# ghy1228/LDPC_Error_Floor

Measured on AMD Instinct MI355X. Metric: decoded codewords/sec, wman N576 R3/4, 20 NMS iters, higher is better.
Workload: dtype i32

## Files before the change

include/ldpc_nms.h:

```cpp
#ifndef LDPC_NMS_H
#define LDPC_NMS_H

#include <stdint.h>

#ifdef __cplusplus
extern "C" {
#endif

#define LDPC_NMS_ABI_VERSION 3

typedef struct ldpc_graph ldpc_graph;
typedef struct ldpc_ctx ldpc_ctx;

enum ldpc_status {
    LDPC_OK = 0,
    LDPC_ERR_ARG = -1,
    LDPC_ERR_HIP = -2,
    LDPC_ERR_OOM = -3,
    LDPC_ERR_STATE = -4,
    LDPC_ERR_UNSUPPORTED = -5
};

enum ldpc_decoding_type {
    LDPC_DEC_SP = 0,
// ... 31 lines not shown
int ldpc_abi_version(void);
const char* ldpc_status_string(int status);

int ldpc_graph_create(const int32_t* proto, int32_t M, int32_t N, int32_t z, int32_t device,
                      ldpc_graph** out);
int ldpc_graph_destroy(ldpc_graph* g);
int ldpc_graph_query(const ldpc_graph* g, int32_t* dims);

int ldpc_weights_set(ldpc_graph* g, int32_t T, const float* alpha, const float* alpha_ucn,
                     const float* beta);

int ldpc_ctx_create(ldpc_graph* g, int64_t B_max, int32_t T_max, ldpc_ctx** out);
int ldpc_ctx_destroy(ldpc_ctx* c);

int ldpc_decode(ldpc_ctx* c, const float* llr_dev, int64_t B, const ldpc_decode_params* p,
                const ldpc_decode_outputs* o, void* stream);

int ldpc_kernel_info(const ldpc_ctx* c, const ldpc_decode_params* p, int64_t* bytes_per_cw,
                     char* name, int32_t name_len);

int ldpc_ctx_last_kernel(const ldpc_ctx* c, char* name, int32_t name_len);

int ldpc_ctx_last_frozen(const ldpc_ctx* c);

int ldpc_channel_awgn(float* llr_dev, int64_t B, int32_t n_vars, double sigma, uint64_t seed,
                      int64_t offset, int32_t decoding_type, int32_t q_bit, int32_t punct_start,
                      int32_t punct_end, int32_t short_start, int32_t short_end, float clip_llr,
                      void* stream);

typedef struct ldpc_channel_params {
    double sigma;
    uint64_t seed;
    int64_t offset;
    int32_t punct_start, punct_end, short_start, short_end;
    int32_t reserved[4];
} ldpc_channel_params;

int ldpc_decode_awgn(ldpc_ctx* ctx, int64_t B, const ldpc_decode_params* params,
                     const ldpc_channel_params* channel, const ldpc_decode_outputs* outputs,
                     void* stream);

int ldpc_awgn_in_kernel(const ldpc_ctx* ctx, const ldpc_decode_params* params, int32_t has_short,
                        int32_t app);

typedef struct ldpc_es_outputs {
    int32_t size;
// ... 101 lines not shown
```

include/ldpc_nms_debug.h:

```cpp
#ifndef LDPC_NMS_DEBUG_H
#define LDPC_NMS_DEBUG_H

#include <stdint.h>

#include "ldpc_nms.h"

#ifdef __cplusplus
extern "C" {
#endif

int ldpc_debug_bs_bounds(const int32_t* proto, int32_t M, int32_t N, int32_t z, int32_t T,
                         int32_t mode, int32_t alpha_uniform, int32_t beta_uniform, float clip,
                         int32_t flags, int32_t* violations, char* msg, int32_t msg_len);

int ldpc_debug_bs_frozen(const int32_t* proto, int32_t M, int32_t N, int32_t z, int32_t T, int32_t mode,
                         int32_t alpha_uniform, int32_t beta_uniform, int32_t ucn, int32_t kind,
                         float clip, int32_t* plan, int32_t* frozen, int32_t n, char* names,
                         int32_t names_len);

int ldpc_debug_events_out(ldpc_ctx* ctx, const uint32_t* planes_dev, const uint32_t* bad_dev, int64_t B,
                          int32_t target_bits, const uint8_t* n_iter_dev, int32_t T,
                          const ldpc_event_outputs* outputs, void* stream);

#ifdef __cplusplus
}
#endif

#endif
```

ldpc_error_floor_amd/csrc/ldpc_bs.hip:

```cpp
#include <algorithm>
#include <array>
#include <cmath>
#include <cstdio>
#include <cstdlib>
#include <cstring>
#include <functional>
#include <string>
#include <utility>
#include <vector>

#include "ldpc_bs_host.h"

namespace ldpc {
namespace bs {

__global__ void k_bs_tables(const float* __restrict__ alpha, const float* __restrict__ alpha_ucn,
                            const float* __restrict__ beta, const int32_t* __restrict__ row_ptr,
                            int T, int E, int N, int arows, int ar, int bcols, float step, float inv,
                            int qmax, float cu, uint32_t* alut, uint32_t* blut) {
    const int f = blockIdx.x * blockDim.x + threadIdx.x;
    const int na = T * ar, nbt = T * bcols;
    if (f >= na + nbt) return;
    int g[16];
    uint32_t* out;
// ... 700 lines not shown
    a.cn_lanes = p.cn_lanes;
    a.cn_dmin = p.cn_dmin;
    a.fold_wave = p.cn_lanes < 64 * p.nw ? (uint32_t)(p.nw - 1) : (p.nw > 1 ? 1u : 0u);
    a.inv = 1.0f / step;
    a.cu = p.cu > 0.f ? p.cu : -1.f;
    a.qmax = bs_qmax(r.mode);
    a.ucn = p.ucn ? 1 : 0;
    a.ucn_iter = g.w_ucn_iter;
    a.beta_id = g.w_beta_id_mask;
    a.row_ptr = g.row_ptr;
    a.z = g.z;
    a.vn_tab = gt;
    const size_t nvt = (size_t)k.VPL * 64 * p.nw * VNW;
    a.vn_wdeg = reinterpret_cast<const int32_t*>(gt + nvt);
    a.row_lay = a.vn_wdeg + 3 * (size_t)k.VPL * p.nw;
    a.cn_chunk = a.row_lay + 2 * (size_t)g.M;
    a.cn_hd = reinterpret_cast<const uint32_t*>(a.cn_chunk + (size_t)p.nw * k.CPL);
    a.alut = alut;
    a.blut = blut;
    a.arows = p.arows;
    a.bcols = p.bcols;
    a.btid = (bs_qmax(r.mode) == QMAX && !getenv("LDPC_BS_NOBFIX")) ? g.beta_tid : nullptr;
    a.btid_n = g.N;
    a.counters = o.counters;
    a.flags = o.flags;
    a.bad = o.bad;
    a.iter_wrong = r.es ? nullptr : b.iter_wrong;
    a.hdx = o.hdx;
    bs_stagger(k.VPL > 1 || k.CPL > 1, &a.stagger, &a.stagger_n);
    a.off_slots = p.off_slots;
    a.off_pad = p.off_pad;
    a.off_zero = p.off_zero;
    a.off_red = p.off_red;
    a.off_alut = p.off_alut;
    a.off_blut = p.off_blut;
    a.off_hdz = p.off_hdz;
    a.off_hdl = p.off_hdl;
    a.off_ch = p.off_ch;
    if (const char* e = getenv("LDPC_DIAG_ABLATE")) a.ablate = atoi(e);
    const int npacks = (int)((b.B + PACK - 1) / PACK);
    int grid = -1;
    if (const char* e = getenv("LDPC_BS_GRID")) grid = std::max(atoi(e), 0);
    a.ticket = nullptr;
    if (bs_loops(k)) {
        const char* e = getenv("LDPC_BS_TICKETS");
        if (e ? atoi(e) != 0 : true) {
// ... 50 lines not shown
            fprintf(f, "bs_wg_launch inst %d T %d B %lld packs %d q8 %d frozen %d tickets %d\n"
                    "# bs_wg wg packs rt_entry rt_exit clk_entry clk_exit hw_id xcc_id   (rt: 100 MHz ticks, clk: shader clocks)\n",
                    p.inst, b.T, (long long)b.B, npacks, b.q8 != nullptr, (int)frozen, tickets);
            for (int w = 0; w < npacks; ++w) {
                const unsigned long long* r = rec.data() + (size_t)BS_WG_REC * w;
                if (!r[0]) continue;
                fprintf(f, "bs_wg %d %llu %llu %llu %llu %llu %08llx %llu\n", w, r[0], r[1], r[2], r[3], r[4],
                        r[5] & 0xFFFFFFFFull, r[5] >> 32);
            }
            fclose(f);
        }
    }
    return st;
#else
    return kLaunch[p.inst](a, npacks, p.nw, lds, s, src, grid, ws.bs_resident);
#endif
}

int bs_decode(const DevGraph& g, const Bufs& b, FusedWorkspace& ws, const float* llr, const BsReq& r,
              const BsOut& o, hipStream_t s) {
    bool to_bsc;
    BsPlan p = bs_route(g, r, &to_bsc);
    ws.bs_frozen = false;
    if (!p.ok) return to_bsc ? bsc_decode(g, b, ws, llr, r, o, s) : LDPC_ERR_UNSUPPORTED;
    const bool frozen = bs_frozen_fit(g, p, r, o.hdx != nullptr || o.hdw != nullptr);
    return bs_run(g, b, ws, p, llr, r, o, frozen, s);
}

}

namespace ldpc {
namespace bs {
struct BoundsReport {
    int violations = 0;
    std::string first;
    void fail(const char* what, long long idx, long long lim) {
        if (violations++ == 0) {
            char buf[160];
            snprintf(buf, sizeof(buf), "%s: index %lld outside [0, %lld)", what, idx, lim);
            first = buf;
        }
    }
    void in(const char* what, long long idx, long long lim) {
        if (idx < 0 || idx >= lim) fail(what, idx, lim);
    }
    void lds(const char* what, long long a, long long n, long long lo, long long hi) {
// ... 238 lines not shown
```

ldpc_error_floor_amd/csrc/ldpc_bs_kernel.h:

```cpp
#pragma once
#include <type_traits>
#include <cstdint>

#include "ldpc_beta_tabs.h"
#include "ldpc_fused.h"
#include "ldpc_fused5_kernel.h"
#include "ldpc_bitplane.h"
#include "ldpc_bs_frozen.h"

namespace ldpc {
namespace bs {

constexpr int PACK = 32;
constexpr int SLOT_W = 5;
constexpr int SLOT_B = SLOT_W * 4;
constexpr int LUT_W = 64;
constexpr int BLUT_W = LUT_W + 4;
constexpr int QMAX = 15;
constexpr size_t BS_LDS_MAX = 160 * 1024;

struct BsInst { int D, DV, LPC, VPL, CPL; bool UCN, BIG, PK; int WPE; bool ES = false; };
constexpr BsInst kBsInst[] = {
    {15, 6, 4, 1, 1, false, false, true, 8},
    {16, 8, 4, 1, 1, false, false, true, 8},
// ... 403 lines not shown
        int la[4];
        awgn_levels4b(g, bucket, thi, tlo, (uint32_t)v, gq, la);
        uint32_t w = word(la);
        if (sh) {
            int lb[4];
            awgn_levels4b(g, bucket, thi, tlo, (uint32_t)v, gq + 1, lb);
            w = __builtin_amdgcn_alignbyte(word(lb), w, (uint32_t)sh);
        }
        D[i] = w;
    }
}
__device__ __forceinline__ void gen_tables(const BsGen& g, int tid, int NT) {
    copy_async(g.lds, g.tab, AWGN_TAB_W, __builtin_amdgcn_readfirstlane(tid >> 6), NT);
}

constexpr double STAGGER_US = 60.0;
constexpr int FLORW = 32;
constexpr bool bs_loops(const BsInst& k) { return k.VPL == 1 && k.CPL == 1 && !k.UCN; }
#if defined(BS_INST) && BS_INST <= 2
#define BS_LOOP_TU 1
#else
#define BS_LOOP_TU 0
#endif
constexpr int BS_RED_NEXT = 8;
#define BS_PACK_SETUP(pk)                                                                          \
    const int64_t b0 = (int64_t)(pk) * PACK;                                                       \
    const int nvalid = (int)min<int64_t>(PACK, a.B - b0);                                          \
    const uint32_t valid = (nvalid >= 32) ? 0xFFFFFFFFu : ((1u << nvalid) - 1u);                   \
    uint32_t* RED = reinterpret_cast<uint32_t*>(smem + (FZ ? W::off_red : a.off_red));             \
    const int flor = 16 + ((a.T + 3) & ~3);                                                        \
    const int AR = UCN ? 2 * (FZ ? W::arows : a.arows) : (FZ ? W::arows : a.arows);                \
    const int AL = AR * LUT_W, BL = (FZ ? W::bcols : a.bcols) * BLUT_W;                            \
    uint32_t* ALUT = reinterpret_cast<uint32_t*>(smem + (FZ ? W::off_alut : a.off_alut));          \
    uint32_t* BLUT = reinterpret_cast<uint32_t*>(smem + (FZ ? W::off_blut : a.off_blut));          \
    const bool ucn = UCN && a.ucn;                                                                 \
    auto ucn_on = [&](int t) __attribute__((always_inline)) -> bool {                              \
        return ucn && (t >= 64 || ((a.ucn_iter >> t) & 1));                                        \
    };

template <int D, int DV, int LPC, int VPL, int CPL, bool UCN, bool BIG, bool PK, int WPE, bool XP, int LB, bool Q8,
          bool ES = false, bool EW = false, bool FZ = false, bool L8 = false>
__global__ void __launch_bounds__(LB) __attribute__((amdgpu_waves_per_eu(WPE)))
k_bs(std::conditional_t<ES, std::conditional_t<EW, BsArgsEw, BsArgsEs>, std::conditional_t<XP, BsArgsXp, BsArgs>> a) {
    static_assert(LPC == 2 || LPC == 4, "lanes per check");
    using KArgs = std::conditional_t<ES, std::conditional_t<EW, BsArgsEw, BsArgsEs>, std::conditional_t<XP, BsArgsXp, BsArgs>>;
    static_assert(!ES || (UCN && VPL == 1 && CPL == 1 && !XP), "early stop: one-chunk UCN-compiled instances");
    static_assert(!EW || ES, "the stop-iteration word: early-stop builds");
    static_assert(!L8 || (!Q8 && !ES && !FZ), "int8 LLRs: the decode and export builds");
    static_assert(!FZ || (BS_LOOP_TU && !UCN && !XP && !ES && VPL == 1 && CPL == 1 && D == 15 && DV == 6 && LPC == 4),
                  "frozen geometry: the wman pack-loop builds");
    using W = BsFrozenWman;
    static_assert(W::cstride == W::z * SLOT_B && W::AL == W::arows * LUT_W && W::BL == W::bcols * BLUT_W &&
                  W::NT == 64 * W::nw && W::off_zero == W::off_pad + SLOT_B, "BsFrozenWman is consistent");
    constexpr int SB = (DV * QMAX + QMAX <= 127) ? 8 : 9;
    constexpr int EPL = (D + LPC - 1) / LPC;
    constexpr bool SKIPM = CPL > 1;
    constexpr int OB = 4 / LPC;
    constexpr int VNA = PK ? (DV + 1) / 2 : DV;
    constexpr int VNW = VNA + 1;
    constexpr int HDW = (EPL + 1) / 2;
    constexpr bool PKG = PK && CPL == 1;
    constexpr bool ONE = VPL == 1 && CPL == 1;
    constexpr int PRIO = ONE ? (DV >= 6 ? 4 : 2) : 0;
    constexpr int PROPRIO = PRIO == 4 ? 3 : 0;
    constexpr bool T0A = ONE;
    constexpr bool EBR = T0A;
    constexpr int SBSET = ONE ? 3 : 2;
    constexpr int KEEP0 = ONE ? 3 : (UCN ? 4 : 7);
    constexpr int KEEP = DV <= 4 ? DV : (KEEP0 < DV ? KEEP0 : DV - 1);
    constexpr bool BKPF = !XP && VPL > 1;
    extern __shared__ __attribute__((aligned(16))) unsigned char smem[];
    if ((uint32_t)(uintptr_t)smem != 0u) __builtin_trap();
#ifdef BS_STAMP
    uint64_t sacc[13] = {};
    uint64_t sts = __builtin_amdgcn_s_memtime();
    if (a.stamps && threadIdx.x == 0) {
        unsigned long long* rec = a.stamps + BS_WG_BASE + (size_t)BS_WG_REC * blockIdx.x;
        rec[1] = __builtin_amdgcn_s_memrealtime();
        rec[3] = sts;
    }
#define BS_ST(i)                                                                                   \
    do {                                                                                           \
        const uint64_t tn_ = __builtin_amdgcn_s_memtime();                                         \
        sacc[i] += tn_ - sts;                                                                      \
        sts = tn_;                                                                                 \
    } while (0)
#else
#define BS_ST(i) ((void)0)
#endif
    const int tid = threadIdx.x;
    const int NT = FZ ? W::NT : (int)blockDim.x;
    const int lane = tid & 63;
    const int wave = __builtin_amdgcn_readfirstlane(tid >> 6);
// ... 511 lines not shown
    const uint32_t cstride = (uint32_t)((FZ ? W::z : a.z) * SLOT_B);
    const uint32_t tabu = (uint32_t)((FZ ? W::arows : a.arows) * LUT_W * 4);
    constexpr bool GBL = CPL == 1;
    if constexpr (GBL) lds_put((FZ ? W::off_ch : a.off_ch) + 4u * (uint32_t)tid, gbase[0]);
    constexpr bool HDL = UCN && CPL == 1;
    if constexpr (HDL) {
#pragma unroll
        for (int p = 0; p < HDW; ++p) lds_put(a.off_hdl + 4u * (uint32_t)(p * NT + tid), ghd[0][p]);
    }
    __syncthreads();

    BS_ST(4);
    for (int t = 0; t < (ABL(16) ? 0 : a.T); ++t) {
        PH("top", 0);
        if (!ONE && wave == 0 && t > 0) {
            const uint32_t ln = __builtin_amdgcn_mbcnt_hi(~0u, __builtin_amdgcn_mbcnt_lo(~0u, 0u));
            uint32_t x = ln < 32u ? RED[flor + ln] : 0u;
            if (ln < 32u) RED[flor + ln] = 0u;
            const uint32_t w0 = wave_or(x);
            RED[16 + t - 1] = w0;
            RED[1] &= w0;
        }
        const int nx = (t + 1) & 1;
#pragma unroll
        for (int u = 0; u < VPL; ++u) asm volatile("" : "+s"(dw[u]), "+s"(dwmin[u]));
        if (!RPW) asm volatile("" : "+s"(cn_dmin));
        const int cdm = FZ ? W::cn_dmin : FOLDB ? (cn_dmin & (FOLDB - 1)) : cn_dmin;
        if (RPW) {
#pragma unroll
            for (int u = 0; u < VPL; ++u) asm volatile("" : "+v"(vv[u]));
        }
        if (t + 1 < a.T) {
            int cw = wave, al = AL, bl = BL, bcl = (FZ ? W::bcols : a.bcols);
            if (!FZ && !(Q8 && VPL == 1 && CPL == 1 && !UCN))
                asm volatile("" : "+s"(cw), "+s"(al), "+s"(bl), "+s"(bcl));
            const uint32_t* alut_p = a.alut;
            const uint32_t* blut_p = a.blut;
            uint32_t off_al = (FZ ? W::off_alut : a.off_alut), off_bl = (FZ ? W::off_blut : a.off_blut);
            if constexpr (VPL == 1 && CPL == 1 && !(Q8 && !UCN)) {
                typedef __attribute__((address_space(4))) const BsArgs ConstArgs;
                ConstArgs* ka = (ConstArgs*)__builtin_amdgcn_kernarg_segment_ptr();
                asm volatile("" : "+s"(ka));
                alut_p = ka->alut;
                blut_p = ka->blut;
                if constexpr (!FZ) {
                    off_al = ka->off_alut;
                    off_bl = ka->off_blut;
                }
            }
            copy_async(off_al + 4u * (uint32_t)(nx * al), alut_p + (size_t)(t + 1) * al, al, cw, NT);
            if (bcl > 1)
                copy_async(off_bl + 4u * (uint32_t)(nx * bl), blut_p + (size_t)(t + 1) * bl, bl, cw, NT);
        }
        if constexpr (BKPF) {
            if (t + 1 < a.T && a.btid) {
#pragma unroll
                for (int u = 0; u < VPL; ++u) {
                    const int col = ((FZ ? W::bcols : a.bcols) == 1) ? 0 : pcol[u];
                    bkp[u] = col >= 0 ? a.btid[(size_t)(t + 1) * (FZ ? W::btid_n : a.btid_n) + col] : -1;
                }
            }
        }
        if (PRIO == 2) __builtin_amdgcn_s_setprio(1);
        if (PRIO == 4) __builtin_amdgcn_s_setprio(2);
#pragma unroll
        for (int c = 0; c < CPL; ++c) {
            const bool active = (CPL == 1) ? (FZ && W::cn_lanes >= W::NT) || wave * 64 < (FZ ? W::cn_lanes : a.cn_lanes) : (gchunk[c] >= 0);
            if (!active || ABL(1)) continue;
            PH("ck_addr", c);
            uint32_t cbase;
            if constexpr (GBL) {
                uint32_t all = ~0u;
                asm volatile("" : "+s"(all));
// ... 71 lines not shown
    case k:                                                                                        \
        if constexpr (k <= EPL) {                                                                  \
            PH("ck_mink", 16 * c + k);                                                             \
            min2_bits<k, LPC>(m1, m2, cand, Xs);                                                   \
            _Pragma("unroll") for (int m = k; m < EPL; ++m) cand[m] = 0u;                          \
        } else {                                                                                   \
            __builtin_unreachable();                                                               \
        }                                                                                          \
        break;
                    BS_MIN2_CASE(1) BS_MIN2_CASE(2) BS_MIN2_CASE(3) BS_MIN2_CASE(4) BS_MIN2_CASE(5)
                    BS_MIN2_CASE(6) BS_MIN2_CASE(7) BS_MIN2_CASE(8)
#undef BS_MIN2_CASE
                    default:
                        __builtin_unreachable();
                }
            } else {
                min2_bits<EPL, LPC>(m1, m2, cand, Xs);
            }
            PH9("ck_merge", c, m1, m2, par);
            par ^= qperm<QP_X1>(par);
            if (LPC == 4) par ^= qperm<QP_X2>(par);
            uint32_t q1[4], q2[4];
            PH9("ck_tab", c, m1, m2, par);
            {
                const uint32_t mm[2][4] = {{m1[0], m1[1], m1[2], m1[3]}, {m2[0], m2[1], m2[2], m2[3]}};
                const uint32_t tab = ctab + (uint32_t)((t & 1) * AL * 4);
                uint32_t qb[OB][2];
                bool any_unsat = false;
                if constexpr (UCN) any_unsat = ucn_t && (CPL == 1 || __builtin_amdgcn_ballot_w64(syn != 0u) != 0ull);
#pragma unroll
                for (int b = 0; b < OB; ++b) {
                    uint32_t o[2];
                    lut_bit<2>(o, mm, tab + (uint32_t)(b * 64));
                    if constexpr (UCN) {
                        if (any_unsat) {
                            uint32_t ou[2];
                            lut_bit<2>(ou, mm, tab + tabu + (uint32_t)(b * 64));
                            o[0] = mux(syn, ou[0], o[0]);
                            o[1] = mux(syn, ou[1], o[1]);
                        }
                    }
                    qb[b][0] = o[0];
                    qb[b][1] = o[1];
                }
                if (LPC == 4) {
                    q1[0] = qperm<0x00>(qb[0][0]); q1[1] = qperm<0x55>(qb[0][0]);
                    q1[2] = qperm<0xAA>(qb[0][0]); q1[3] = qperm<0xFF>(qb[0][0]);
// ... 187 lines not shown
#pragma unroll
        for (int i = 0; i < 13; ++i) atomicAdd(a.stamps + 16 * wave + i, (unsigned long long)sacc[i]);
        atomicAdd(a.stamps + 16 * wave + 15, npk);
        uint32_t hw;
        asm volatile("s_getreg_b32 %0, hwreg(HW_REG_HW_ID)" : "=s"(hw));
        const uint32_t simd = (((hw >> 4) & 3u) - reinterpret_cast<uint32_t*>(smem + (FZ ? W::off_red : a.off_red))[12]) & 3u;
        atomicAdd(a.stamps + 16 * wave + 13 + (simd >> 1), npk << (32 * (simd & 1)));
        if (wave == 0) {
            uint32_t xcc;
            asm volatile("s_getreg_b32 %0, hwreg(HW_REG_XCC_ID)" : "=s"(xcc));
            unsigned long long* rec = a.stamps + BS_WG_BASE + (size_t)BS_WG_REC * blockIdx.x;
            rec[0] = npk;
            rec[2] = __builtin_amdgcn_s_memrealtime();
            rec[4] = __builtin_amdgcn_s_memtime();
            rec[5] = (unsigned long long)xcc << 32 | hw;
        }
    }
#endif
#undef BS_ST
}

struct BsLaunch : BsArgsEw {
    int word;
    bool frozen;
    uint32_t* ticket;
};

template <class K>
K kernel_arg_of(void (*)(K));
template <class K, class L>
K bs_kernel_args(const L& a) {
    if constexpr (std::is_base_of_v<K, L>) return a;
    else return K{a, a.word};
}
template <auto Fn>
void bs_max_lds() {
    static const hipError_t once = hipFuncSetAttribute(reinterpret_cast<const void*>(Fn),
                                                       hipFuncAttributeMaxDynamicSharedMemorySize, (int)BS_LDS_MAX);
    (void)once;
}
template <auto Fn, class L>
int bs_launch_kernel(const L& a, int nblocks, int nw, size_t lds, hipStream_t s) {
    bs_max_lds<Fn>();
    hipLaunchKernelGGL(Fn, dim3(nblocks), dim3(64 * nw), lds, s, bs_kernel_args<decltype(kernel_arg_of(Fn))>(a));
    return hipGetLastError() == hipSuccess ? LDPC_OK : LDPC_ERR_HIP;
}

template <int I, bool XP, bool Q8, bool FZ = false, bool L8 = false>
int launch_bs_x(const BsLaunch& a, int npacks, int nw, size_t lds, hipStream_t s, int grid, int* resident) {
    constexpr BsInst k = kBsInst[I];
    static_assert(bs_loops(k) == (BS_LOOP_TU != 0), "BS_LOOP_TU lists the instances of bs_loops");
    constexpr auto fn = &k_bs<k.D, k.DV, k.LPC, k.VPL, k.CPL, k.UCN, k.BIG, k.PK, k.WPE, XP, 1024, Q8, false, false, FZ, L8>;
    int nblocks = npacks;
    if constexpr (bs_loops(k)) {
        if (grid < 0) {
// ... 69 lines not shown
```

ldpc_error_floor_amd/csrc/ldpc_capi.hip:

```cpp
#include <cstdio>
#include <cstring>
#include <functional>
#include <new>
#include <vector>

#include "ldpc_awgn.h"
#include "ldpc_internal.h"
#include "ldpc_fused.h"

using namespace ldpc;

struct ldpc_graph {
    int device = 0;
    host::GraphTables h;
    int32_t* d_tables = nullptr;
    DevGraph dev{};
    int T_w = 0;
    int per_edge_w = 0;
    std::vector<int32_t> row_merge;
    int32_t* d_row_merge = nullptr;
    float* d_alpha = nullptr;
    float* d_alpha_ucn = nullptr;
    float* d_beta = nullptr;
    int32_t* d_beta_tid = nullptr;
};

struct ldpc_ctx {
    ldpc_graph* g = nullptr;
    int64_t B_max = 0;
    int T_max = 0;
    int ntiles_max = 0;
    float* ch = nullptr;
    float* Tv = nullptr;
    float* c2v = nullptr;
    uint64_t* hd = nullptr;
    uint64_t* wrong = nullptr;
    uint64_t* anypos = nullptr;
    int32_t* biterr = nullptr;
    FusedWorkspace fused{};
    float* llr_scratch = nullptr;
    int64_t llr_scratch_n = 0;
    uint32_t* gen_tab = nullptr;
    uint32_t gen_host[AWGN_TAB_W] = {};
    bool gen_valid = false;
    hipEvent_t gen_done = nullptr;
    bool gen_pending = false;
    char last_kernel[64] = {0};
// ... 214 lines not shown
    d.n_checks = M * z; d.n_vars = N * z; d.n_edges = h.E * z; d.max_cdeg = h.max_cdeg;
    const int32_t* p = g->d_tables;
    d.row_ptr = p; p += M + 1;
    d.pe_row = p; p += h.E;
    d.pe_col = p; p += h.E;
    d.pe_shift = p; p += h.E;
    d.col_ptr = p; p += N + 1;
    d.col_pe = p;
    d.vn_edge = reinterpret_cast<const int4*>(g->d_tables + h.off_vn);
    d.h_row_ptr = h.row_ptr.data();
    d.host = &g->h;
    *out = g;
    return LDPC_OK;
}

int ldpc_graph_destroy(ldpc_graph* g) {
    if (!g) return LDPC_ERR_ARG;
    DeviceGuard dg(g->device);
    dev_free(g->d_tables);
    dev_free(g->d_alpha);
    dev_free(g->d_alpha_ucn);
    dev_free(g->d_beta);
    dev_free(g->d_beta_tid);
    dev_free(g->d_row_merge);
    delete g;
    return LDPC_OK;
}

int ldpc_graph_query(const ldpc_graph* g, int32_t* dims) {
    if (!g || !dims) return LDPC_ERR_ARG;
    const host::GraphTables& h = g->h;
    const int32_t v[8] = {h.M, h.N, h.z, h.E, h.M * h.z, h.N * h.z, h.E * h.z, h.max_cdeg};
    std::memcpy(dims, v, sizeof(v));
    return LDPC_OK;
}

int ldpc_weights_set(ldpc_graph* g, int32_t T, const float* alpha, const float* alpha_ucn,
                     const float* beta) {
    if (!g) return LDPC_ERR_ARG;
    if (alpha && alpha_ucn && T > 0 && g->h.E > 0 &&
        std::memcmp(alpha, alpha_ucn, (size_t)T * g->h.E * sizeof(float)) == 0)
        alpha_ucn = nullptr;
    host::WeightInfo wi;
    const int sta = host::analyze_weights(g->h, T, alpha, alpha_ucn, beta, wi);
    if (sta != LDPC_OK) return sta;
    DeviceGuard dg(g->device);
    dev_free(g->d_alpha);
    dev_free(g->d_alpha_ucn);
    dev_free(g->d_beta);
    dev_free(g->d_beta_tid);
    g->dev.beta_tid = nullptr;
    g->T_w = 0;
    const size_t ne = (size_t)T * g->h.E, nn = (size_t)T * g->h.N;
    int st = dev_alloc(&g->d_alpha, ne);
    if (st == LDPC_OK && alpha_ucn) st = dev_alloc(&g->d_alpha_ucn, ne);
    if (st == LDPC_OK) st = dev_alloc(&g->d_beta, nn);
    if (st == LDPC_OK) st = dev_alloc(&g->d_beta_tid, nn);
    if (st != LDPC_OK) return st;
    bool ok = hipMemcpy(g->d_alpha, alpha, ne * sizeof(float), hipMemcpyHostToDevice) == hipSuccess;
    if (alpha_ucn)
        ok = ok && hipMemcpy(g->d_alpha_ucn, alpha_ucn, ne * sizeof(float),
                             hipMemcpyHostToDevice) == hipSuccess;
    ok = ok && hipMemcpy(g->d_beta, beta, nn * sizeof(float), hipMemcpyHostToDevice) == hipSuccess;
    ok = ok && hipMemcpy(g->d_beta_tid, wi.beta_tid.data(), nn * sizeof(int32_t), hipMemcpyHostToDevice) == hipSuccess;
    if (!ok) return LDPC_ERR_HIP;
    g->dev.beta_tid = g->d_beta_tid;
    g->T_w = T;
    g->per_edge_w = wi.per_edge_w;
    g->row_merge = wi.row_merge;
    g->dev.h_row_merge = nullptr;
    g->dev.row_merge = nullptr;
    if (!g->d_row_merge) {
        const int st2 = dev_alloc(&g->d_row_merge, (size_t)g->h.M);
        if (st2 != LDPC_OK) return st2;
    }
    if (hipMemcpy(g->d_row_merge, g->row_merge.data(), (size_t)g->h.M * sizeof(int32_t),
                  hipMemcpyHostToDevice) != hipSuccess)
        return LDPC_ERR_HIP;
    g->dev.h_row_merge = g->row_merge.data();
    g->dev.row_merge = g->d_row_merge;
    g->dev.w_alpha_uniform = wi.alpha_uniform;
    g->dev.w_alpha_pair_uniform = wi.alpha_pair_uniform;
    g->dev.w_beta_uniform = wi.beta_uniform;
    g->dev.w_beta_nonneg = wi.beta_nonneg;
    g->dev.w_beta_one = wi.beta_one;
    g->dev.w_beta_id_mask = wi.beta_id_mask;
    g->dev.w_ucn_iter = wi.ucn_iter_mask;
    g->dev.w_version++;
    return LDPC_OK;
// ... 531 lines not shown
    if (!o->early_stop) return LDPC_ERR_UNSUPPORTED;
    const EventSink ev = event_sink(o, ch->offset, p);
    return decode_awgn_es_impl(c, B, p, ch, bs_outs(o, &ev), stream);
}

int ldpc_debug_events_out(ldpc_ctx* c, const uint32_t* planes_dev, const uint32_t* bad_dev, int64_t B,
                          int32_t target_bits, const uint8_t* n_iter_dev, int32_t T, const ldpc_event_outputs* o,
                          void* stream) {
    if (!event_outputs_ok(o)) return LDPC_ERR_ARG;
    if (!c || !planes_dev || !bad_dev || B <= 0 || target_bits < 0) return LDPC_ERR_ARG;
    ldpc_graph* g = c->g;
    if (target_bits > g->h.N * g->h.z) return LDPC_ERR_ARG;
    DeviceGuard dg(g->device);
    const EventSink ev{o->frame_base, o->cap, o->ev_count, o->ev_frame, o->ev_info, o->ev_word, target_bits};
    return events_out(g->dev, planes_dev, bad_dev, B, n_iter_dev, T, ev, o->frame_flags,
                      reinterpret_cast<hipStream_t>(stream));
}

int ldpc_ctx_last_frozen(const ldpc_ctx* c) {
    if (!c) return LDPC_ERR_ARG;
    return (c->fused.bs_frozen && std::strncmp(c->last_kernel, "bsl[", 4) == 0) ? 1 : 0;
}

int ldpc_ctx_last_kernel(const ldpc_ctx* c, char* name, int32_t name_len) {
    if (!c || !name || name_len <= 0) return LDPC_ERR_ARG;
    std::strncpy(name, c->last_kernel, (size_t)name_len - 1);
    name[name_len - 1] = 0;
    return LDPC_OK;
}

}
```

ldpc_error_floor_amd/csrc/ldpc_fused.h:

```cpp
#pragma once
#include <string>

#include "ldpc_internal.h"

namespace ldpc {

struct FusedWorkspace {
    uint64_t* hd = nullptr;
    int64_t hd_elems = 0;
    void* tables = nullptr;
    size_t tables_bytes = 0;
    void* bs_graph = nullptr;
    int bs_graph_inst = -1;
    void* bs_es_graph = nullptr;
    int bs_es_graph_inst = -1;
    void* bs_lut = nullptr;
    size_t bs_lut_bytes = 0;
    uint32_t* bs_bad = nullptr;
    int64_t bs_bad_n = 0;
    int bs_resident[7] = {0, 0, 0, 0, 0, 0, 0};
    uint64_t bs_resident_key = ~0ull;
    uint32_t* bs_ticket = nullptr;
    bool bs_frozen = false;
    uint32_t* hdx = nullptr;
    int64_t hdx_elems = 0;
    bool bits_packed = false;
    uint32_t* hdw = nullptr;
    int64_t hdw_elems = 0;
    uint8_t* ev_niter = nullptr;
    int64_t ev_niter_n = 0;
    const char* last_kernel = "";
    uint64_t key_gad[4] = {~0ull, 0, 0, 0}, key_qtab[4] = {~0ull, 0, 0, 0}, key_bslut[4] = {~0ull, 0, 0, 0};
};

template <class T, class N>
int dev_grow(T*& p, N& have, size_t n, size_t elem) {
    if ((size_t)have >= n) return LDPC_OK;
    if (p) (void)hipFree(p);
    p = nullptr;
    have = 0;
    if (hipMalloc(reinterpret_cast<void**>(&p), n * elem) != hipSuccess) {
        (void)hipGetLastError();
        return LDPC_ERR_OOM;
    }
    have = (N)n;
    return LDPC_OK;
// ... 88 lines not shown
```

ldpc_error_floor_amd/csrc/ldpc_host.cpp:

```cpp
#include "ldpc_host.h"
#include "ldpc_beta_tabs.h"

#include <algorithm>
#include <climits>
#include <cmath>

namespace ldpc {
namespace host {

int build_graph(const int32_t* proto, int32_t M, int32_t N, int32_t z, GraphTables& g) {
    g = GraphTables{};
    if (!proto || M <= 0 || N <= 0 || z <= 0) return LDPC_ERR_ARG;
    if ((int64_t)M * N * z > INT32_MAX) return LDPC_ERR_ARG;
    g.M = M;
    g.N = N;
    g.z = z;
    g.row_ptr.assign((size_t)M + 1, 0);
    for (int i = 0; i < M; ++i)
        for (int j = 0; j < N; ++j) {
            const int32_t s = proto[(size_t)i * N + j];
            if (s < -1) return LDPC_ERR_ARG;
            if (s != -1) {
                g.pe_row.push_back(i);
                g.pe_col.push_back(j);
// ... 32 lines not shown
        const int pe = g.col_pe[(size_t)e], i = g.pe_row[(size_t)pe], r0 = g.row_ptr[(size_t)i];
        h.push_back(r0 * z + (pe - r0));
        h.push_back(g.row_ptr[(size_t)i + 1] - r0);
        h.push_back(g.pe_shift[(size_t)pe]);
        h.push_back(((i * z) << 6) | (pe - r0));
    }
    return LDPC_OK;
}

int beta_table_id(float b) {
    if (!(b >= 0.f)) return -1;
    uint8_t t[16];
    for (int m = 0; m < 16; ++m)
        t[m] = (uint8_t)std::min(15.f, std::fabs(std::nearbyint((float)m * b)));
    int lo = 0, hi = kNBetaTab;
    int sum = 0;
    for (int m = 0; m < 16; ++m) sum += t[m];
    for (int k = lo; k < hi; ++k) {
        int s = 0;
        for (int m = 0; m < 16; ++m) s += kBetaTab[k][m];
        if (s != sum) continue;
        if (std::equal(t, t + 16, kBetaTab[k])) return k;
    }
    return -1;
}

int analyze_weights(const GraphTables& g, int32_t T, const float* alpha, const float* alpha_ucn,
                    const float* beta, WeightInfo& w) {
    w = WeightInfo{};
    if (T <= 0 || !alpha || !beta || g.E <= 0) return LDPC_ERR_ARG;
    if ((int64_t)T * g.E > INT32_MAX || (int64_t)T * g.N > INT32_MAX) return LDPC_ERR_ARG;
    for (int t = 0; t < T && !w.per_edge_w; ++t)
        for (int i = 0; i < g.M && !w.per_edge_w; ++i)
            for (int e = g.row_ptr[(size_t)i] + 1; e < g.row_ptr[(size_t)i + 1]; ++e) {
                const size_t a0 = (size_t)t * g.E + g.row_ptr[(size_t)i], a1 = (size_t)t * g.E + e;
                if (alpha[a1] != alpha[a0] || (alpha_ucn && alpha_ucn[a1] != alpha_ucn[a0])) {
                    w.per_edge_w = 1;
                    break;
                }
            }
    w.row_merge.assign((size_t)g.M, 0);
    for (int i = 1; i < g.M && !w.per_edge_w; ++i) {
        const int deg = g.row_ptr[(size_t)i + 1] - g.row_ptr[(size_t)i];
        bool same = deg == g.row_ptr[(size_t)i] - g.row_ptr[(size_t)i - 1];
        for (int t = 0; t < T && same && deg > 0; ++t) {
            const size_t a0 = (size_t)t * g.E + g.row_ptr[(size_t)i - 1];
// ... 24 lines not shown
        }
        if (id) w.beta_id_mask |= (uint64_t)1 << t;
    }
    if (alpha_ucn)
        for (int t = 0; t < T && t < 64; ++t)
            for (int e = 0; e < g.E; ++e)
                if (alpha_ucn[(size_t)t * g.E + e] != alpha[(size_t)t * g.E + e]) {
                    w.ucn_iter_mask |= (uint64_t)1 << t;
                    break;
                }
    w.beta_tid.resize((size_t)T * g.N);
    for (size_t x = 0; x < (size_t)T * g.N; ++x) w.beta_tid[x] = beta_table_id(beta[x]);
    for (int t = 0; t < T; ++t) {
        const float a0 = alpha[(size_t)t * g.E], b0 = beta[(size_t)t * g.N];
        for (int e = 1; e < g.E && w.alpha_uniform; ++e)
            if (alpha[(size_t)t * g.E + e] != a0) w.alpha_uniform = 0;
        for (int j = 0; j < g.N; ++j) {
            const float b = beta[(size_t)t * g.N + j];
            if (b != b0) w.beta_uniform = 0;
            if (!(b >= 0.f)) w.beta_nonneg = 0;
            if (b != 1.f) w.beta_one = 0;
        }
    }
    return LDPC_OK;
}

int check_decode(const GraphTables& g, int64_t B, int64_t B_max, int32_t T_max, int32_t T_w,
                 const ldpc_decode_params* p, int* mode) {
    if (!p) return LDPC_ERR_ARG;
    if (B <= 0 || B > B_max || p->T <= 0 || p->T > T_max) return LDPC_ERR_STATE;
    if (T_w < p->T) return LDPC_ERR_STATE;
    const int m = mode_of(p->decoding_type, p->q_bit);
    if (m < 0) return LDPC_ERR_ARG;
    if (p->target_bits <= 0 || p->target_bits > g.N * g.z) return LDPC_ERR_ARG;
    if (!(p->clip_llr > 0.f) || !std::isfinite(p->clip_llr)) return LDPC_ERR_ARG;
    if (p->kernel != LDPC_KERNEL_AUTO && p->kernel != LDPC_KERNEL_FLOOD &&
        p->kernel != LDPC_KERNEL_FUSED)
        return LDPC_ERR_ARG;
    if (mode) *mode = m;
    return LDPC_OK;
}

int check_channel(int64_t B, int32_t n_vars, double sigma, int64_t offset, int32_t decoding_type,
                  int32_t q_bit, int32_t punct_start, int32_t punct_end, int32_t short_start,
                  int32_t short_end, float clip_llr) {
    if (B <= 0 || n_vars <= 0 || !(sigma > 0.0) || !std::isfinite(sigma) || offset < 0)
// ... 95 lines not shown
```

ldpc_error_floor_amd/csrc/ldpc_host.h:

```cpp
#pragma once
#include <cstddef>
#include <cstdint>
#include <utility>
#include <vector>

#include "ldpc_nms.h"

namespace ldpc {

enum Mode : int { MODE_Q6 = 0, MODE_Q5, MODE_QM5, MODE_Q4, MODE_Q3, MODE_MS, MODE_MSNN, MODE_SP };
constexpr bool mode_is_qms(int m) { return m >= 0 && m <= MODE_Q3; }

inline int mode_of(int decoding_type, int q_bit) {
    if (decoding_type == LDPC_DEC_SP) return MODE_SP;
    if (decoding_type == LDPC_DEC_MS) return MODE_MS;
    if (decoding_type == LDPC_DEC_MS_NONUDGE) return MODE_MSNN;
    if (decoding_type != LDPC_DEC_QMS) return -1;
    switch (q_bit) {
        case 6: return MODE_Q6;
        case 5: return MODE_Q5;
        case -5: return MODE_QM5;
        case 4: return MODE_Q4;
        case 3: return MODE_Q3;
        default: return -1;
    }
}

namespace host {

constexpr int kMaxCheckDegree = 64;

struct GraphTables {
    int M = 0, N = 0, z = 0, E = 0;
    int max_cdeg = 0, max_vdeg = 0;
    std::vector<int32_t> row_ptr;
    std::vector<int32_t> pe_row;
    std::vector<int32_t> pe_col;
    std::vector<int32_t> pe_shift;
    std::vector<int32_t> col_ptr;
    std::vector<int32_t> col_pe;
    std::vector<int32_t> device_block;
    size_t off_vn = 0;
};

int build_graph(const int32_t* proto, int32_t M, int32_t N, int32_t z, GraphTables& out);

struct WeightInfo {
    int per_edge_w = 0;
    int alpha_uniform = 0, beta_uniform = 0, beta_nonneg = 0, beta_one = 0;
    int alpha_pair_uniform = 0;
    uint64_t beta_id_mask = 0;
    uint64_t ucn_iter_mask = 0;
    std::vector<int32_t> row_merge;
    std::vector<int32_t> beta_tid;
};
int beta_table_id(float beta);
int analyze_weights(const GraphTables& g, int32_t T, const float* alpha, const float* alpha_ucn,
                    const float* beta, WeightInfo& out);

int check_decode(const GraphTables& g, int64_t B, int64_t B_max, int32_t T_max, int32_t T_w,
                 const ldpc_decode_params* p, int* mode);

int check_channel(int64_t B, int32_t n_vars, double sigma, int64_t offset, int32_t decoding_type,
                  int32_t q_bit, int32_t punct_start, int32_t punct_end, int32_t short_start,
                  int32_t short_end, float clip_llr);

std::pair<int, int> order_variable_edges(std::vector<uint32_t>& A, const std::vector<int>& deg, int DV,
                                         int rounds);

void awgn_qms_levels(double sigma, int q_bit, int* nb, int* kmin, uint32_t* thr_hi, uint32_t* thr_lo,
                     float* val);

}
}
```

ldpc_error_floor_amd/csrc/pybind_module.cpp:

```cpp
#include <pybind11/numpy.h>
#include <pybind11/pybind11.h>

#include <algorithm>
#include <stdexcept>
#include <string>

#include "ldpc_nms.h"
#include "ldpc_nms_debug.h"

namespace py = pybind11;

static void check(int st, const char* what) {
    if (st < 0)
        throw std::runtime_error(std::string(what) + ": " + ldpc_status_string(st) + " (" +
                                 std::to_string(st) + ")");
}

struct Graph {
    ldpc_graph* h = nullptr;
    explicit Graph(py::array_t<int32_t, py::array::c_style | py::array::forcecast> proto, int z,
                   int device) {
        if (proto.ndim() != 2) throw std::invalid_argument("proto must be 2-D");
        check(ldpc_graph_create(proto.data(), (int32_t)proto.shape(0), (int32_t)proto.shape(1), z,
                                device, &h),
// ... 530 lines not shown
            check(r < 0 ? r : 0, "ldpc_awgn_in_kernel");
            return r == 1;
        },
        py::arg("ctx"), py::arg("T"), py::arg("decoding_type"), py::arg("q_bit"),
        py::arg("target_bits"), py::arg("kernel"), py::arg("clip_llr") = 20.0f,
        py::arg("has_short") = false, py::arg("app") = false);
    m.def(
        "last_kernel",
        [](Ctx& c) {
            char name[64] = {0};
            check(ldpc_ctx_last_kernel(c.h, name, 64), "ldpc_ctx_last_kernel");
            return std::string(name);
        },
        py::arg("ctx"));
    m.def(
        "last_frozen",
        [](Ctx& c) {
            const int r = ldpc_ctx_last_frozen(c.h);
            check(r < 0 ? r : 0, "ldpc_ctx_last_frozen");
            return r == 1;
        },
        py::arg("ctx"));
    m.def(
        "format_uncor_rows",
        [](py::array_t<float, py::array::c_style | py::array::forcecast> rows) {
            if (rows.ndim() != 2 || rows.shape(1) <= 0)
                throw std::invalid_argument("rows must be [n, n_cols] with n_cols > 0");
            const int64_t n = rows.shape(0), nc = rows.shape(1);
            const int64_t step = std::max<int64_t>(1, (64 << 20) / LDPC_UNCOR_ROW_BOUND(nc));
            std::string out, buf;
            out.reserve((size_t)(n * (12 + 6 * nc)));
            buf.resize((size_t)(std::min(n, step) * LDPC_UNCOR_ROW_BOUND(nc)));
            {
                py::gil_scoped_release nogil;
                for (int64_t r0 = 0; r0 < n; r0 += step) {
                    const int64_t k = std::min(step, n - r0);
                    int64_t len = 0;
                    check(ldpc_format_uncor_rows(rows.data() + r0 * nc, k, nc, buf.data(),
                                                 (int64_t)buf.size(), &len),
                          "ldpc_format_uncor_rows");
                    out.append(buf.data(), (size_t)len);
                }
            }
            return py::bytes(out);
        },
        py::arg("rows"));
// ... 2 lines not shown
```

ldpc_error_floor_amd/decoder.py:

```python
from __future__ import annotations

from dataclasses import dataclass
from typing import Optional

import numpy as np

from . import _native
from .code import TannerGraph
from .config import DECODING_MS, DECODING_MS_NONUDGE, DECODING_QMS, DECODING_SP, VALID_Q_BITS
from .weights import DecoderWeights

__all__ = ["NMSDecoder", "Decoder", "DecodeResult", "KERNELS"]

KERNELS = {"auto": 0, "flood": 1, "fused": 2}
Q8_GRIDS = {5: (0.5, 15), -5: (1.0, 15), 4: (1.0, 7), 3: (2.0, 3)}


@dataclass
class DecodeResult:
    app: Optional["object"] = None
    hard: Optional["object"] = None
    synd: Optional["object"] = None
    counters: Optional["object"] = None
    flags: Optional["object"] = None
# ... 528 lines not shown
              out.numel() < B * self.n_vars):
            raise ValueError("out must be a contiguous int8 [B, N*z] tensor on the decoder's device")
        if stream is None:
            stream = torch.cuda.current_stream(self.device)
        self._ext.channel_awgn_q8(out.data_ptr(), int(B), self.n_vars, float(sigma), int(seed), int(offset),
                                  self.q_bit, int(punct[0]), int(punct[1]), int(short[0]), int(short[1]),
                                  stream.cuda_stream)
        return out

    def generates_channel_in_kernel(self, T=None, kernel=None, app: bool = False) -> bool:
        T = self.T if T is None else T
        ctx = self._ensure_ctx(1, T)
        short = getattr(self, "short", (0, 0)) or (0, 0)
        return bool(self._ext.awgn_in_kernel(ctx, T, self.decoding_type, self.q_bit, self.target_bits,
                                             KERNELS[kernel or self.kernel], self.clip,
                                             has_short=short[0] > 0, app=app))

    def last_kernel(self) -> str:
        return "" if self._ctx is None else self._ext.last_kernel(self._ctx)

    def last_frozen(self) -> bool:
        return False if self._ctx is None else bool(self._ext.last_frozen(self._ctx))

    def _empty_result(self, T, nt, hard, synd, counters, flags, app, iter_wrong=False):
        torch = self._torch
        dev = self.device
        res = DecodeResult()
        if app:
            res.app = torch.empty((T, 0, nt), dtype=torch.float32, device=dev)
        if hard:
            res.hard = torch.empty((T, 0, (self.n_vars + 31) // 32), dtype=torch.int32, device=dev)
        if synd:
            res.synd = torch.empty((T, 0, (self.n_checks + 31) // 32), dtype=torch.int32, device=dev)
        if counters is True:
            counters = torch.zeros(4, dtype=torch.int64, device=dev)
        res.counters = counters if counters is not None else None
        if isinstance(flags, torch.Tensor):
            res.flags = flags[:0]
        elif flags:
            res.flags = torch.empty(0, dtype=torch.uint8, device=dev)
        if iter_wrong:
            res.iter_wrong = torch.empty((T, 0), dtype=torch.int32, device=dev)
        return res

    def decode_awgn(self, B: int, sigma: float, seed: int, offset: int = 0, punct=None, short=None,
                    T: Optional[int] = None, app: bool = False, counters=None, flags=None,
# ... 172 lines not shown
```

Measured before the change: 303.4 million.

## Use fixed beta-table asm path for uniform alpha in bit-sliced loop kernel

When alpha is uniform per iteration and matches one of the precomputed 16-entry quantized tables, the host records a table id per iteration and passes it to the bit-sliced loop kernel. The kernel then applies the scaling through the hardcoded beta_asm path instead of async-copying per-iteration alpha LUTs into shared memory and doing table lookups. This cuts LDS traffic and lookup work in the check-node update. The cost is an extra kernarg pointer, a per-iteration scalar load, and a new template path that only applies to one-chunk, non-UCN Q5/QM5 instances.

```diff
diff --git a/include/ldpc_nms.h b/include/ldpc_nms.h
--- a/include/ldpc_nms.h
+++ b/include/ldpc_nms.h
@@ -77,6 +77,8 @@
 int ldpc_ctx_last_kernel(const ldpc_ctx* c, char* name, int32_t name_len);
 
 int ldpc_ctx_last_frozen(const ldpc_ctx* c);
+
+int ldpc_ctx_last_afix(const ldpc_ctx* c);
 
 int ldpc_channel_awgn(float* llr_dev, int64_t B, int32_t n_vars, double sigma, uint64_t seed,
                       int64_t offset, int32_t decoding_type, int32_t q_bit, int32_t punct_start,
diff --git a/include/ldpc_nms_debug.h b/include/ldpc_nms_debug.h
--- a/include/ldpc_nms_debug.h
+++ b/include/ldpc_nms_debug.h
@@ -18,6 +18,11 @@
                          float clip, int32_t* plan, int32_t* frozen, int32_t n, char* names,
                          int32_t names_len);
 
+int ldpc_debug_alpha_tid(float alpha, int32_t mode, int32_t* out_id, uint8_t* table);
+
+int ldpc_debug_alpha_tids(const int32_t* proto, int32_t M, int32_t N, int32_t z, int32_t T,
+                          const float* alpha, const float* alpha_ucn, int32_t* ids);
+
 int ldpc_debug_events_out(ldpc_ctx* ctx, const uint32_t* planes_dev, const uint32_t* bad_dev, int64_t B,
                           int32_t target_bits, const uint8_t* n_iter_dev, int32_t T,
                           const ldpc_event_outputs* outputs, void* stream);
diff --git a/ldpc_error_floor_amd/csrc/ldpc_bs.hip b/ldpc_error_floor_amd/csrc/ldpc_bs.hip
--- a/ldpc_error_floor_amd/csrc/ldpc_bs.hip
+++ b/ldpc_error_floor_amd/csrc/ldpc_bs.hip
@@ -746,6 +746,12 @@
     a.bcols = p.bcols;
     a.btid = (bs_qmax(r.mode) == QMAX && !getenv("LDPC_BS_NOBFIX")) ? g.beta_tid : nullptr;
     a.btid_n = g.N;
+    a.atid = nullptr;
+    if (bs_loops(k) && !p.ucn && p.arows == 1 && (r.mode == MODE_Q5 || r.mode == MODE_QM5)) {
+        const char* e = getenv("LDPC_BS_AFIX");
+        if (e ? atoi(e) != 0 : true) a.atid = g.host->w_alpha_tid_dev;
+    }
+    ws.bs_afix = a.atid != nullptr;
     a.counters = o.counters;
     a.flags = o.flags;
     a.bad = o.bad;
@@ -842,6 +848,7 @@
     bool to_bsc;
     BsPlan p = bs_route(g, r, &to_bsc);
     ws.bs_frozen = false;
+    ws.bs_afix = false;
     if (!p.ok) return to_bsc ? bsc_decode(g, b, ws, llr, r, o, s) : LDPC_ERR_UNSUPPORTED;
     const bool frozen = bs_frozen_fit(g, p, r, o.hdx != nullptr || o.hdw != nullptr);
     return bs_run(g, b, ws, p, llr, r, o, frozen, s);
diff --git a/ldpc_error_floor_amd/csrc/ldpc_bs_kernel.h b/ldpc_error_floor_amd/csrc/ldpc_bs_kernel.h
--- a/ldpc_error_floor_amd/csrc/ldpc_bs_kernel.h
+++ b/ldpc_error_floor_amd/csrc/ldpc_bs_kernel.h
@@ -449,6 +449,12 @@
 #else
 #define BS_LOOP_TU 0
 #endif
+template <class K>
+struct BsArgsAf : K {
+    const int32_t* atid;
+};
+template <class K>
+using BsKernArgs = std::conditional_t<BS_LOOP_TU != 0, BsArgsAf<K>, K>;
 constexpr int BS_RED_NEXT = 8;
 #define BS_PACK_SETUP(pk)                                                                          \
     const int64_t b0 = (int64_t)(pk) * PACK;                                                       \
@@ -468,7 +474,7 @@
 template <int D, int DV, int LPC, int VPL, int CPL, bool UCN, bool BIG, bool PK, int WPE, bool XP, int LB, bool Q8,
           bool ES = false, bool EW = false, bool FZ = false, bool L8 = false>
 __global__ void __launch_bounds__(LB) __attribute__((amdgpu_waves_per_eu(WPE)))
-k_bs(std::conditional_t<ES, std::conditional_t<EW, BsArgsEw, BsArgsEs>, std::conditional_t<XP, BsArgsXp, BsArgs>> a) {
+k_bs(BsKernArgs<std::conditional_t<ES, std::conditional_t<EW, BsArgsEw, BsArgsEs>, std::conditional_t<XP, BsArgsXp, BsArgs>>> a) {
     static_assert(LPC == 2 || LPC == 4, "lanes per check");
     using KArgs = std::conditional_t<ES, std::conditional_t<EW, BsArgsEw, BsArgsEs>, std::conditional_t<XP, BsArgsXp, BsArgs>>;
     static_assert(!ES || (UCN && VPL == 1 && CPL == 1 && !XP), "early stop: one-chunk UCN-compiled instances");
@@ -496,6 +502,8 @@
     constexpr int KEEP0 = ONE ? 3 : (UCN ? 4 : 7);
     constexpr int KEEP = DV <= 4 ? DV : (KEEP0 < DV ? KEEP0 : DV - 1);
     constexpr bool BKPF = !XP && VPL > 1;
+    constexpr bool AFX = BS_LOOP_TU != 0;
+    static_assert(!AFX || (ONE && !UCN), "fixed-set check tables: the one-chunk instances without UCN");
     extern __shared__ __attribute__((aligned(16))) unsigned char smem[];
     if ((uint32_t)(uintptr_t)smem != 0u) __builtin_trap();
 #ifdef BS_STAMP
@@ -1053,6 +1061,16 @@
             RED[1] &= w0;
         }
         const int nx = (t + 1) & 1;
+        int ak = 0;
+        bool afx = false;
+        if constexpr (AFX) {
+            typedef __attribute__((address_space(4))) const BsArgsAf<KArgs> ConstAf;
+            ConstAf* kq = (ConstAf*)__builtin_amdgcn_kernarg_segment_ptr();
+            asm volatile("" : "+s"(kq));
+            const ConstW* at = (const ConstW*)kq->atid;
+            afx = at != nullptr;
+            if (afx) ak = (int)at[t];
+        }
 #pragma unroll
         for (int u = 0; u < VPL; ++u) asm volatile("" : "+s"(dw[u]), "+s"(dwmin[u]));
         if (!RPW) asm volatile("" : "+s"(cn_dmin));
@@ -1079,7 +1097,8 @@
                     off_bl = ka->off_blut;
                 }
             }
-            copy_async(off_al + 4u * (uint32_t)(nx * al), alut_p + (size_t)(t + 1) * al, al, cw, NT);
+            if (!(AFX && afx))
+                copy_async(off_al + 4u * (uint32_t)(nx * al), alut_p + (size_t)(t + 1) * al, al, cw, NT);
             if (bcl > 1)
                 copy_async(off_bl + 4u * (uint32_t)(nx * bl), blut_p + (size_t)(t + 1) * bl, bl, cw, NT);
         }
@@ -1197,7 +1216,10 @@
             if (LPC == 4) par ^= qperm<QP_X2>(par);
             uint32_t q1[4], q2[4];
             PH9("ck_tab", c, m1, m2, par);
-            {
+            if (AFX && afx) {
+                beta_asm(q1, m1, ak);
+                beta_asm(q2, m2, ak);
+            } else {
                 const uint32_t mm[2][4] = {{m1[0], m1[1], m1[2], m1[3]}, {m2[0], m2[1], m2[2], m2[3]}};
                 const uint32_t tab = ctab + (uint32_t)((t & 1) * AL * 4);
                 uint32_t qb[OB][2];
@@ -1431,15 +1453,22 @@
 
 struct BsLaunch : BsArgsEw {
     int word;
+    const int32_t* atid;
     bool frozen;
     uint32_t* ticket;
 };
 
 template <class K>
 K kernel_arg_of(void (*)(K));
+template <class K>
+struct BsAfBase { using type = void; };
+template <class K>
+struct BsAfBase<BsArgsAf<K>> { using type = K; };
 template <class K, class L>
 K bs_kernel_args(const L& a) {
     if constexpr (std::is_base_of_v<K, L>) return a;
+    else if constexpr (!std::is_void_v<typename BsAfBase<K>::type>)
+        return K{bs_kernel_args<typename BsAfBase<K>::type>(a), a.atid};
     else return K{a, a.word};
 }
 template <auto Fn>
diff --git a/ldpc_error_floor_amd/csrc/ldpc_capi.hip b/ldpc_error_floor_amd/csrc/ldpc_capi.hip
--- a/ldpc_error_floor_amd/csrc/ldpc_capi.hip
+++ b/ldpc_error_floor_amd/csrc/ldpc_capi.hip
@@ -1,3 +1,4 @@
+#include <algorithm>
 #include <cstdio>
 #include <cstring>
 #include <functional>
@@ -5,6 +6,7 @@
 #include <vector>
 
 #include "ldpc_awgn.h"
+#include "ldpc_beta_tabs.h"
 #include "ldpc_internal.h"
 #include "ldpc_fused.h"
 
@@ -23,6 +25,7 @@
     float* d_alpha_ucn = nullptr;
     float* d_beta = nullptr;
     int32_t* d_beta_tid = nullptr;
+    int32_t* d_alpha_tid = nullptr;
 };
 
 struct ldpc_ctx {
@@ -283,6 +286,7 @@
     dev_free(g->d_alpha_ucn);
     dev_free(g->d_beta);
     dev_free(g->d_beta_tid);
+    dev_free(g->d_alpha_tid);
     dev_free(g->d_row_merge);
     delete g;
     return LDPC_OK;
@@ -310,13 +314,18 @@
     dev_free(g->d_alpha_ucn);
     dev_free(g->d_beta);
     dev_free(g->d_beta_tid);
+    dev_free(g->d_alpha_tid);
     g->dev.beta_tid = nullptr;
+    g->h.w_alpha_tid_dev = nullptr;
     g->T_w = 0;
     const size_t ne = (size_t)T * g->h.E, nn = (size_t)T * g->h.N;
     int st = dev_alloc(&g->d_alpha, ne);
     if (st == LDPC_OK && alpha_ucn) st = dev_alloc(&g->d_alpha_ucn, ne);
     if (st == LDPC_OK) st = dev_alloc(&g->d_beta, nn);
     if (st == LDPC_OK) st = dev_alloc(&g->d_beta_tid, nn);
+    const bool afix = !wi.alpha_tid.empty() &&
+                      std::all_of(wi.alpha_tid.begin(), wi.alpha_tid.end(), [](int32_t k) { return k >= 0; });
+    if (st == LDPC_OK && afix) st = dev_alloc(&g->d_alpha_tid, (size_t)T);
     if (st != LDPC_OK) return st;
     bool ok = hipMemcpy(g->d_alpha, alpha, ne * sizeof(float), hipMemcpyHostToDevice) == hipSuccess;
     if (alpha_ucn)
@@ -324,8 +333,11 @@
                              hipMemcpyHostToDevice) == hipSuccess;
     ok = ok && hipMemcpy(g->d_beta, beta, nn * sizeof(float), hipMemcpyHostToDevice) == hipSuccess;
     ok = ok && hipMemcpy(g->d_beta_tid, wi.beta_tid.data(), nn * sizeof(int32_t), hipMemcpyHostToDevice) == hipSuccess;
+    if (afix)
+        ok = ok && hipMemcpy(g->d_alpha_tid, wi.alpha_tid.data(), (size_t)T * sizeof(int32_t), hipMemcpyHostToDevice) == hipSuccess;
     if (!ok) return LDPC_ERR_HIP;
     g->dev.beta_tid = g->d_beta_tid;
+    g->h.w_alpha_tid_dev = afix ? g->d_alpha_tid : nullptr;
     g->T_w = T;
     g->per_edge_w = wi.per_edge_w;
     g->row_merge = wi.row_merge;
@@ -903,6 +915,34 @@
     return (c->fused.bs_frozen && std::strncmp(c->last_kernel, "bsl[", 4) == 0) ? 1 : 0;
 }
 
+extern "C" int ldpc_debug_alpha_tid(float alpha, int32_t mode, int32_t* out_id, uint8_t* table) {
+    if (!out_id) return LDPC_ERR_ARG;
+    const int k = host::alpha_table_id(alpha, mode);
+    *out_id = k;
+    if (k >= 0 && table) std::memcpy(table, kBetaTab[k], 16);
+    return LDPC_OK;
+}
+
+extern "C" int ldpc_debug_alpha_tids(const int32_t* proto, int32_t M, int32_t N, int32_t z, int32_t T, const float* alpha,
+                          const float* alpha_ucn, int32_t* ids) {
+    if (!proto || !alpha || !ids || T <= 0) return LDPC_ERR_ARG;
+    host::GraphTables h;
+    int st = host::build_graph(proto, M, N, z, h);
+    if (st != LDPC_OK) return st;
+    const std::vector<float> beta((size_t)T * h.N, 1.0f);
+    host::WeightInfo wi;
+    st = host::analyze_weights(h, T, alpha, alpha_ucn, beta.data(), wi);
+    if (st != LDPC_OK) return st;
+    if (wi.alpha_tid.empty()) return 0;
+    std::copy(wi.alpha_tid.begin(), wi.alpha_tid.end(), ids);
+    return 1;
+}
+
+int ldpc_ctx_last_afix(const ldpc_ctx* c) {
+    if (!c) return LDPC_ERR_ARG;
+    return (c->fused.bs_afix && std::strncmp(c->last_kernel, "bsl[", 4) == 0) ? 1 : 0;
+}
+
 int ldpc_ctx_last_kernel(const ldpc_ctx* c, char* name, int32_t name_len) {
     if (!c || !name || name_len <= 0) return LDPC_ERR_ARG;
     std::strncpy(name, c->last_kernel, (size_t)name_len - 1);
diff --git a/ldpc_error_floor_amd/csrc/ldpc_fused.h b/ldpc_error_floor_amd/csrc/ldpc_fused.h
--- a/ldpc_error_floor_amd/csrc/ldpc_fused.h
+++ b/ldpc_error_floor_amd/csrc/ldpc_fused.h
@@ -22,6 +22,7 @@
     uint64_t bs_resident_key = ~0ull;
     uint32_t* bs_ticket = nullptr;
     bool bs_frozen = false;
+    bool bs_afix = false;
     uint32_t* hdx = nullptr;
     int64_t hdx_elems = 0;
     bool bits_packed = false;
diff --git a/ldpc_error_floor_amd/csrc/ldpc_host.cpp b/ldpc_error_floor_amd/csrc/ldpc_host.cpp
--- a/ldpc_error_floor_amd/csrc/ldpc_host.cpp
+++ b/ldpc_error_floor_amd/csrc/ldpc_host.cpp
@@ -78,6 +78,26 @@
         if (s != sum) continue;
         if (std::equal(t, t + 16, kBetaTab[k])) return k;
     }
+    return -1;
+}
+
+static void alpha_table(float alpha, float step, uint8_t (&t)[16]) {
+    const float inv = 1.0f / step;
+    for (int m = 0; m < 16; ++m) {
+        const float mv = (float)m * step;
+        float x = mv * alpha;
+        x = (x > 0.f) ? x : 0.f;
+        const float r = std::nearbyint(x * inv);
+        t[m] = (uint8_t)std::min(std::max(r, -15.f), 15.f);
+    }
+}
+
+int alpha_table_id(float alpha, int mode) {
+    if (mode != MODE_Q5 && mode != MODE_QM5) return -1;
+    uint8_t t[16];
+    alpha_table(alpha, mode == MODE_Q5 ? 0.5f : 1.0f, t);
+    for (int k = 0; k < kNBetaTab; ++k)
+        if (std::equal(t, t + 16, kBetaTab[k])) return k;
     return -1;
 }
 
@@ -148,6 +168,14 @@
             if (b != 1.f) w.beta_one = 0;
         }
     }
+    if (w.alpha_uniform) {
+        w.alpha_tid.resize((size_t)T);
+        for (int t = 0; t < T; ++t) {
+            const float a0 = alpha[(size_t)t * g.E];
+            const int k = alpha_table_id(a0, MODE_Q5);
+            w.alpha_tid[(size_t)t] = (k == alpha_table_id(a0, MODE_QM5)) ? k : -1;
+        }
+    }
     return LDPC_OK;
 }
 
diff --git a/ldpc_error_floor_amd/csrc/ldpc_host.h b/ldpc_error_floor_amd/csrc/ldpc_host.h
--- a/ldpc_error_floor_amd/csrc/ldpc_host.h
+++ b/ldpc_error_floor_amd/csrc/ldpc_host.h
@@ -41,6 +41,7 @@
     std::vector<int32_t> col_pe;
     std::vector<int32_t> device_block;
     size_t off_vn = 0;
+    const int32_t* w_alpha_tid_dev = nullptr;
 };
 
 int build_graph(const int32_t* proto, int32_t M, int32_t N, int32_t z, GraphTables& out);
@@ -53,8 +54,10 @@
     uint64_t ucn_iter_mask = 0;
     std::vector<int32_t> row_merge;
     std::vector<int32_t> beta_tid;
+    std::vector<int32_t> alpha_tid;
 };
 int beta_table_id(float beta);
+int alpha_table_id(float alpha, int mode);
 int analyze_weights(const GraphTables& g, int32_t T, const float* alpha, const float* alpha_ucn,
                     const float* beta, WeightInfo& out);
 
diff --git a/ldpc_error_floor_amd/csrc/pybind_module.cpp b/ldpc_error_floor_amd/csrc/pybind_module.cpp
--- a/ldpc_error_floor_amd/csrc/pybind_module.cpp
+++ b/ldpc_error_floor_amd/csrc/pybind_module.cpp
@@ -576,6 +576,14 @@
         },
         py::arg("ctx"));
     m.def(
+        "last_afix",
+        [](Ctx& c) {
+            const int r = ldpc_ctx_last_afix(c.h);
+            check(r < 0 ? r : 0, "ldpc_ctx_last_afix");
+            return r == 1;
+        },
+        py::arg("ctx"));
+    m.def(
         "format_uncor_rows",
         [](py::array_t<float, py::array::c_style | py::array::forcecast> rows) {
             if (rows.ndim() != 2 || rows.shape(1) <= 0)
diff --git a/ldpc_error_floor_amd/decoder.py b/ldpc_error_floor_amd/decoder.py
--- a/ldpc_error_floor_amd/decoder.py
+++ b/ldpc_error_floor_amd/decoder.py
@@ -574,6 +574,9 @@
     def last_frozen(self) -> bool:
         return False if self._ctx is None else bool(self._ext.last_frozen(self._ctx))
 
+    def last_afix(self) -> bool:
+        return False if self._ctx is None else bool(self._ext.last_afix(self._ctx))
+
     def _empty_result(self, T, nt, hard, synd, counters, flags, app, iter_wrong=False):
         torch = self._torch
         dev = self.device
```

Result: faster. 315.2 million, median of 6 (+3.9%).
